# ayotoasset/AdditiveCausalExpansion

Hardware: AMD Instinct MI355X
Metric: log-marg-lik+grad evals/sec at n=16384,d=20; Cholesky GF/s vs MFMA peak (higher is better)
Workload: dtype f64; 1 GPU; C2: n=16384, d=20, Matern32, ns basis B=10, fp64; one para_update (kernel assembly + SPD inverse/log-det + all P gradients + RMSE/evidence + Nadam step) per step; n=16384, p=20, B=10, kernel=Matern32, parallelism=single

## Files before the change

additivecausalexpansion_amd/csrc/ace_sweep.hip:

```cpp
#include "ace_internal.h"

#include "ace_wgtime.h"

namespace ace {

#define CHAIN_PRIO() __builtin_amdgcn_s_setprio(1)


struct PivotLds {
  __attribute__((aligned(16))) double colb[2][SUB];
  __attribute__((aligned(16))) double rowb[2][SUB];
  double pv[SUB];
};

template <int T>
__device__ __forceinline__ double row_bcast(double x) {
  long v = __builtin_bit_cast(long, x);
  long b = __builtin_amdgcn_update_dpp((long)0, v, 0x150 + T, 0xf, 0xf, true);
  return __builtin_bit_cast(double, b);
}

template <int G>
__device__ __forceinline__ double rep_row_bp(double x, int lane) {
  const int addr = ((lane & 15) | (G << 4)) << 2;
// ... 407 lines not shown
      __hip_atomic_fetch_add(ctr + 1, 1, __ATOMIC_RELAXED, __HIP_MEMORY_SCOPE_AGENT) == nwg - 1) {
    __hip_atomic_store(ctr, 0, __ATOMIC_RELAXED, __HIP_MEMORY_SCOPE_AGENT);
    __hip_atomic_store(ctr + 1, 0, __ATOMIC_RELAXED, __HIP_MEMORY_SCOPE_AGENT);
  }
}

#ifndef ACE_BK
#define ACE_BK 16
#endif
constexpr int BK = ACE_BK;
constexpr int LDL = 144;
constexpr int NCH = NB / BK;
constexpr int UTHREADS = 512;
constexpr int SM128 = 2, SH128 = 64;
constexpr int SM64 = 2, SH64 = 32;
static_assert(BK == 16, "staging maps 512 threads x 4 doubles onto a 128 x 16 chunk");

__device__ __forceinline__ void st_a(double *p, double v) { __builtin_nontemporal_store(v, p); }
__device__ __forceinline__ double ld_a(const double *p) { return __builtin_nontemporal_load(p); }

struct GatherOut {
  double *P, *W, *S0;
  int64_t k0, ldp;
  double *low = nullptr, *send = nullptr;
  int64_t h = 0;
  int G = 1;
  int64_t lr0 = 0;
};
static inline GatherOut no_gather() { return GatherOut{nullptr, nullptr, nullptr, -1, 0}; }
static inline GatherOut pack_out(double *low, double *send, double *P, double *W, double *S0,
                                 int64_t k0, int64_t naug, int G) {
  GatherOut g{P, W, S0, k0, naug};
  if (G > 1) {
    g.low = low;
    g.send = send;
  }
  g.h = naug - k0;
  g.G = G;
  return g;
}

__device__ __forceinline__ void gput(const GatherOut &g, int64_t r, int64_t c, double v) {
  if (r < c) return;
  const int64_t cc = c - g.k0, rr = r - g.k0;
  if (g.low) {
    if ((uint64_t)cc < (uint64_t)NB) {
      g.low[(rr - g.lr0) + cc * g.h] = v;
      if ((uint64_t)rr < (uint64_t)NB && r != c) g.low[cc + rr * g.h] = v;
    } else if ((uint64_t)rr < (uint64_t)NB) {
      g.send[(lcol(c, g.G) / NB) * NB * NB + rr + (c % NB) * NB] = v;
    }
  }
  if (!g.P) return;
  if ((uint64_t)cc < (uint64_t)NB) {
    g.P[r + cc * g.ldp] = -v;
    if ((uint64_t)rr < (uint64_t)NB) {
      g.W[r + cc * g.ldp] = v;
      if (rr < SUB) g.S0[rr + cc * SUB] = v;
    }
  }
  if ((uint64_t)rr < (uint64_t)NB && r != c) {
    g.P[c + rr * g.ldp] = -v;
    if ((uint64_t)cc < (uint64_t)NB) {
      g.W[c + rr * g.ldp] = v;
      if (cc < SUB) g.S0[cc + rr * SUB] = v;
    }
  }
}

__device__ __forceinline__ void gput_aug_dead(const GatherOut &g, const double *A, int64_t ld,
                                              int64_t R0, int64_t C0, int tid, int nthr,
                                              int64_t L0 = -1) {
  const int64_t cc0 = C0 - g.k0;
  if ((uint64_t)cc0 >= (uint64_t)NB) return;
  const int64_t lc0 = L0 >= 0 ? L0 : C0;
  for (int e = tid; e < (UT - 16) * UT; e += nthr) {
    const int a = 16 + e % (UT - 16), c = e / (UT - 16);
    const double v = A[(R0 + a) + (lc0 + c) * ld];
    if (g.low) g.low[(R0 + a - g.k0 - g.lr0) + (cc0 + c) * g.h] = v;
    if (g.P) g.P[(R0 + a) + (cc0 + c) * g.ldp] = -v;
  }
}

__global__ __launch_bounds__(UTHREADS, 2) void k_update(double *__restrict__ A, int64_t ld,
                                                        const double *__restrict__ Rop,
                                                        const double *__restrict__ Cop,
                                                        const double *__restrict__ Wk,
                                                        int64_t ldp, int64_t k0, int kx,
                                                        const Tile *__restrict__ tiles, int G,
                                                        GatherOut go) {
  ACE_WGT(6, gridDim.x < 4096 || blockIdx.x % 32 == 0);
  __shared__ __attribute__((aligned(16))) double sW[2][BK][LDL];
  __shared__ __attribute__((aligned(16))) double sP[2][BK][LDL];
  constexpr int KT = NB / UT;
  int I, J;
  if (tiles) {
    const Tile tt = tiles[blockIdx.x];
    I = tt.I;
    J = tt.J;
    if (I < 0) return;
  } else {
    const int t = blockIdx.x;
    int i = (int)((sqrt(8.0 * (double)t + 1.0) - 1.0) * 0.5);
    while ((i + 1) * (i + 2) / 2 <= t) ++i;
    while (i * (i + 1) / 2 > t) --i;
    I = i;
    J = t - i * (i + 1) / 2;
  }
  if (kx >= 0 && ((I >= kx * KT && I < (kx + 1) * KT) || (J >= kx * KT && J < (kx + 1) * KT)))
    return;
  const int kt0 = (int)(k0 / UT), kt1 = kt0 + KT;
  const bool Ik = I >= kt0 && I < kt1, Jk = J >= kt0 && J < kt1;
  const int64_t R0 = (int64_t)I * UT, C0 = (int64_t)J * UT;
  const int64_t L0 = lcol(C0, G);
  const int tid = threadIdx.x;

  if (Ik || Jk) {
    if (Ik && !Jk) {
      double *tileT = &sW[0][0][0];
      for (int sa = 0; sa < 2; ++sa)
        for (int sb = 0; sb < 2; ++sb) {
          __syncthreads();
          for (int e = tid; e < 4096; e += UTHREADS) {
            const int c = e & 63, a = e >> 6;
            tileT[a * 65 + c] = Wk[(C0 + 64 * sb + c) + (R0 - k0 + 64 * sa + a) * ldp];
          }
          __syncthreads();
          for (int e = tid; e < 4096; e += UTHREADS) {
            const int a = e & 63, c = e >> 6;
            const double v = tileT[a * 65 + c];
            A[(R0 + 64 * sa + a) + (L0 + 64 * sb + c) * ld] = v;
            if (go.k0 >= 0) gput(go, R0 + 64 * sa + a, C0 + 64 * sb + c, v);
          }
        }
    } else {
      for (int e = tid; e < UT * UT; e += UTHREADS) {
        const int a = e & (UT - 1), c = e >> 7;
        const double v = Wk[(R0 + a) + (C0 - k0 + c) * ldp];
        A[(R0 + a) + (L0 + c) * ld] = v;
        if (go.k0 >= 0) gput(go, R0 + a, C0 + c, v);
      }
    }
    return;
  }

  const int lane = tid & 63, wv = tid >> 6;
  const int lr = lane & 15, lk = lane >> 4;
  if (R0 >= ld - AUG) {
    d4 acc;
    const int64_t r = R0 + lr;
    const int64_t c = L0 + 16 * wv + lk;
#pragma unroll
    for (int j = 0; j < 4; ++j) acc[j] = ld_a(&A[r + (c + 4 * j) * ld]);
    const double *gr = Rop + R0 + lr + (int64_t)lk * ldp;
    const double *gc = Cop + C0 + 16 * wv + lr + (int64_t)lk * ldp;
    double an = gc[0], bn = gr[0];
    for (int kk = 0; kk < NB / 4; ++kk) {
      const double a = an, bb = bn;
      if (kk + 1 < NB / 4) {
        an = gc[(int64_t)(4 * (kk + 1)) * ldp];
        bn = gr[(int64_t)(4 * (kk + 1)) * ldp];
      }
      acc = __builtin_amdgcn_mfma_f64_16x16x4f64(a, bb, acc, 0, 0, 0);
    }
#pragma unroll
    for (int j = 0; j < 4; ++j) st_a(&A[r + (c + 4 * j) * ld], acc[j]);
    if (go.k0 >= 0) {
#pragma unroll
      for (int j = 0; j < 4; ++j) gput(go, r, C0 + 16 * wv + lk + 4 * j, acc[j]);
      gput_aug_dead(go, A, ld, R0, C0, tid, UTHREADS, L0);
    }
    return;
  }
  const int sk = tid >> 5, sm = (tid & 31) * SM128;
  const int roff = (int)((R0 + sm) + (int64_t)sk * ldp), coff = (int)((C0 + sm) + (int64_t)sk * ldp);
  double2 rw[2], rp[2];
#pragma unroll
  for (int e = 0; e < 2; ++e) {
    rw[e] = *reinterpret_cast<const double2 *>(Rop + roff + SH128 * e);
    rp[e] = *reinterpret_cast<const double2 *>(Cop + coff + SH128 * e);
  }
  __builtin_amdgcn_sched_barrier(0);
  const int wr = wv & 1, wc = wv >> 1;
  d4 acc[2][4];
#pragma unroll
  for (int ci = 0; ci < 2; ++ci)
#pragma unroll
    for (int ri = 0; ri < 4; ++ri) {
      const int64_t r = R0 + 64 * wr + 16 * ri + lr;
      const int64_t c = L0 + 32 * wc + 16 * ci + lk;
#pragma unroll
      for (int j = 0; j < 4; ++j) acc[ci][ri][j] = ld_a(&A[r + (c + 4 * j) * ld]);
    }
#pragma unroll
  for (int e = 0; e < 2; ++e) {
    *reinterpret_cast<double2 *>(&sW[0][sk][sm + SH128 * e]) = rw[e];
    *reinterpret_cast<double2 *>(&sP[0][sk][sm + SH128 * e]) = rp[e];
  }
  __syncthreads();
  for (int ch = 0; ch < NCH; ++ch) {
    const int cur = ch & 1;
    if (ch + 1 < NCH) {
      const int64_t off = (int64_t)(ch + 1) * BK * ldp;
      const double *nw = Rop + off, *np = Cop + off;
#pragma unroll
      for (int e = 0; e < 2; ++e) {
        rw[e] = *reinterpret_cast<const double2 *>(nw + roff + SH128 * e);
        rp[e] = *reinterpret_cast<const double2 *>(np + coff + SH128 * e);
      }
    }
#pragma unroll
    for (int kk = 0; kk < BK / 4; ++kk) {
      double a[2], b[4];
#pragma unroll
      for (int ci = 0; ci < 2; ++ci) a[ci] = sP[cur][4 * kk + lk][32 * wc + 16 * ci + lr];
#pragma unroll
      for (int ri = 0; ri < 4; ++ri) b[ri] = sW[cur][4 * kk + lk][64 * wr + 16 * ri + lr];
#pragma unroll
      for (int ci = 0; ci < 2; ++ci)
#pragma unroll
        for (int ri = 0; ri < 4; ++ri)
          acc[ci][ri] = __builtin_amdgcn_mfma_f64_16x16x4f64(a[ci], b[ri], acc[ci][ri], 0, 0, 0);
    }
    if (ch + 1 < NCH) {
#pragma unroll
      for (int e = 0; e < 2; ++e) {
        *reinterpret_cast<double2 *>(&sW[cur ^ 1][sk][sm + SH128 * e]) = rw[e];
        *reinterpret_cast<double2 *>(&sP[cur ^ 1][sk][sm + SH128 * e]) = rp[e];
      }
    }
    __syncthreads();
  }
#pragma unroll
  for (int ci = 0; ci < 2; ++ci)
#pragma unroll
    for (int ri = 0; ri < 4; ++ri) {
      const int64_t r = R0 + 64 * wr + 16 * ri + lr;
      const int64_t c = L0 + 32 * wc + 16 * ci + lk;
#pragma unroll
      for (int j = 0; j < 4; ++j) st_a(&A[r + (c + 4 * j) * ld], acc[ci][ri][j]);
    }
  if (go.k0 >= 0) {
#pragma unroll
    for (int ci = 0; ci < 2; ++ci)
#pragma unroll
      for (int ri = 0; ri < 4; ++ri)
#pragma unroll
        for (int j = 0; j < 4; ++j)
          gput(go, R0 + 64 * wr + 16 * ri + lr, C0 + 32 * wc + 16 * ci + lk + 4 * j, acc[ci][ri][j]);
  }
}

__global__ __launch_bounds__(UTHREADS, 2) void k_panel_gemm_t(double *__restrict__ W,
                                                              const double *__restrict__ Pn,
                                                              int64_t ldp, int64_t k0, int G,
                                                              int r, int rt0 = 0,
                                                              int rs0 = 1 << 30, int rs1 = 1 << 30) {
  ACE_WGT(3, true);
  __shared__ __attribute__((aligned(16))) double sW[2][BK][LDL];
  __shared__ __attribute__((aligned(16))) double sP[2][BK][LDL];
  int rt = rt0 + (int)blockIdx.x;
  if (rt >= rs0) rt += rs1 - rs0;
  const int64_t R0 = (int64_t)rt * UT, C0 = (int64_t)blockIdx.y * UT;
  if (R0 >= k0 && R0 < k0 + NB) return;
  if (G > 1 && !owns_col(R0, G, r) && !(owns_col(k0, G, r) && R0 >= k0)) return;
  const int tid = threadIdx.x, lane = tid & 63, wv = tid >> 6;
  const int lr = lane & 15, lk = lane >> 4;
  const int sk = tid >> 5, sm = (tid & 31) * SM128;
  const double *gW = Pn + (R0 + sm) + (int64_t)sk * ldp;
  const double *gP = W + (k0 + C0 + sm) + (int64_t)sk * ldp;
  const int wr = wv & 1, wc = wv >> 1;
  d4 acc[2][4];
#pragma unroll
  for (int ci = 0; ci < 2; ++ci)
#pragma unroll
    for (int ri = 0; ri < 4; ++ri) acc[ci][ri] = d4{0.0, 0.0, 0.0, 0.0};
  double2 w00, w01, p00, p01;
#define PG_LOAD(W0, W1, P0, P1, CH)                                               \
  do {                                                                            \
    const int64_t off_ = (int64_t)(CH) * BK * ldp;                                \
    W0 = *reinterpret_cast<const double2 *>(gW + off_);                           \
    W1 = *reinterpret_cast<const double2 *>(gW + off_ + SH128);                   \
    P0 = *reinterpret_cast<const double2 *>(gP + off_);                           \
    P1 = *reinterpret_cast<const double2 *>(gP + off_ + SH128);                   \
  } while (0)
#define PG_STAGE(W0, W1, P0, P1, BUF)                                             \
  do {                                                                            \
    *reinterpret_cast<double2 *>(&sW[BUF][sk][sm]) = W0;                          \
    *reinterpret_cast<double2 *>(&sW[BUF][sk][sm + SH128]) = W1;                  \
    *reinterpret_cast<double2 *>(&sP[BUF][sk][sm]) = P0;                          \
    *reinterpret_cast<double2 *>(&sP[BUF][sk][sm + SH128]) = P1;                  \
  } while (0)
  auto mma = [&](int cur) {
#pragma unroll
    for (int kk = 0; kk < BK / 4; ++kk) {
      double a[2], b[4];
#pragma unroll
      for (int ci = 0; ci < 2; ++ci) a[ci] = sP[cur][4 * kk + lk][32 * wc + 16 * ci + lr];
#pragma unroll
      for (int ri = 0; ri < 4; ++ri) b[ri] = sW[cur][4 * kk + lk][64 * wr + 16 * ri + lr];
#pragma unroll
      for (int ci = 0; ci < 2; ++ci)
#pragma unroll
        for (int ri = 0; ri < 4; ++ri)
          acc[ci][ri] = __builtin_amdgcn_mfma_f64_16x16x4f64(a[ci], b[ri], acc[ci][ri], 0, 0, 0);
    }
  };
  {
    PG_LOAD(w00, w01, p00, p01, 0);
    PG_STAGE(w00, w01, p00, p01, 0);
    __syncthreads();
    ACE_WGT_MARK(0);
    for (int ch = 0; ch < NCH; ++ch) {
      const int cur = ch & 1;
      if (ch + 1 < NCH) PG_LOAD(w00, w01, p00, p01, ch + 1);
      mma(cur);
      if (ch + 1 < NCH) PG_STAGE(w00, w01, p00, p01, cur ^ 1);
      __syncthreads();
    }
  }
#undef PG_LOAD
#undef PG_STAGE
  ACE_WGT_MARK(1);
#pragma unroll
  for (int ci = 0; ci < 2; ++ci)
#pragma unroll
    for (int ri = 0; ri < 4; ++ri) {
      const int64_t rr = R0 + 64 * wr + 16 * ri + lr;
      const int64_t c = C0 + 32 * wc + 16 * ci + lk;
#pragma unroll
      for (int j = 0; j < 4; ++j) W[rr + (c + 4 * j) * ldp] = acc[ci][ri][j];
    }
}

struct PanelSet {
  const double *R[4];
  const double *C[4];
};
__device__ __forceinline__ const double *psel(const double *const (&p)[4], int j) {
  return j == 0 ? p[0] : j == 1 ? p[1] : j == 2 ? p[2] : p[3];
}

template <bool SH, bool OPQ = false>
__device__ __forceinline__ void update_multi_tile(int I, int J, double (&sW)[2][BK][LDL],
                                                  double (&sP)[2][BK][LDL], double *__restrict__ A,
                                                  int64_t ld, const PanelSet &ps, int npan,
                                                  int64_t ldp, int64_t ka0, const GatherOut &go,
                                                  int G) {
  constexpr int KT = NB / UT;
  const int ta0 = (int)(ka0 / UT);
  const int di = I - ta0, dj = J - ta0;
  const int bi = (di >= 0 && di < npan * KT) ? di / KT : -1;
  const int bj = (dj >= 0 && dj < npan * KT) ? dj / KT : -1;
  const int jm = bi > bj ? bi : bj;
  const int64_t R0 = (int64_t)I * UT, C0 = (int64_t)J * UT;
  const int64_t L0 = SH ? lcol(C0, G) : C0;
  int tid = threadIdx.x;
  if (OPQ) __asm__ volatile("" : "+v"(tid));
  const double *const(&WS)[4] = SH ? ps.C : ps.R;

  if (jm == npan - 1) {
    const double *Wl = psel(WS, jm);
    const int64_t kl0 = ka0 + (int64_t)jm * NB;
    if (bi == jm && bj != jm) {
      double *tileT = &sW[0][0][0];
      for (int sa = 0; sa < 2; ++sa)
        for (int sb = 0; sb < 2; ++sb) {
          __syncthreads();
          for (int e = tid; e < 4096; e += UTHREADS) {
            const int c = e & 63, a = e >> 6;
            tileT[a * 65 + c] = Wl[(C0 + 64 * sb + c) + (R0 - kl0 + 64 * sa + a) * ldp];
          }
          __syncthreads();
          for (int e = tid; e < 4096; e += UTHREADS) {
            const int a = e & 63, c = e >> 6;
            const double v = tileT[a * 65 + c];
            A[(R0 + 64 * sa + a) + (L0 + 64 * sb + c) * ld] = v;
            if (go.k0 >= 0) gput(go, R0 + 64 * sa + a, C0 + 64 * sb + c, v);
          }
        }
    } else {
      for (int e = tid; e < UT * UT; e += UTHREADS) {
        const int a = e & (UT - 1), c = e >> 7;
        const double v = Wl[(R0 + a) + (C0 - kl0 + c) * ldp];
        A[(R0 + a) + (L0 + c) * ld] = v;
        if (go.k0 >= 0) gput(go, R0 + a, C0 + c, v);
      }
    }
    return;
  }
  const bool from_w = jm >= 0;
  const int seg0 = from_w ? jm + 1 : 0;
  const bool jin = bj == jm;
  const int64_t wrs = jin ? 1 : ldp, wcs = jin ? ldp : 1;
  const double *wab = from_w ? psel(WS, jm) - (ka0 + (int64_t)jm * NB) * ldp : nullptr;

  const int lane = tid & 63, wv = tid >> 6;
  const int lr = lane & 15, lk = lane >> 4;
  if (R0 >= ld - AUG) {
    d4 acc;
    const int64_t r = R0 + lr;
    const int64_t c = C0 + 16 * wv + lk, lc = L0 + 16 * wv + lk;
#pragma unroll
    for (int j = 0; j < 4; ++j)
      acc[j] = from_w ? wab[r * wrs + (c + 4 * j) * wcs] : ld_a(&A[r + (lc + 4 * j) * ld]);
    for (int pnl = seg0; pnl < npan; ++pnl) {
      const double *gr = psel(ps.R, pnl) + R0 + lr + (int64_t)lk * ldp;
      const double *gc = psel(ps.C, pnl) + C0 + 16 * wv + lr + (int64_t)lk * ldp;
      double an = gc[0], bn = gr[0];
      for (int kk = 0; kk < NB / 4; ++kk) {
        const double a = an, bb = bn;
        if (kk + 1 < NB / 4) {
          an = gc[(int64_t)(4 * (kk + 1)) * ldp];
          bn = gr[(int64_t)(4 * (kk + 1)) * ldp];
        }
        acc = __builtin_amdgcn_mfma_f64_16x16x4f64(a, bb, acc, 0, 0, 0);
      }
    }
#pragma unroll
    for (int j = 0; j < 4; ++j) st_a(&A[r + (lc + 4 * j) * ld], acc[j]);
    if (go.k0 >= 0) {
#pragma unroll
      for (int j = 0; j < 4; ++j) gput(go, r, c + 4 * j, acc[j]);
      gput_aug_dead(go, A, ld, R0, C0, tid, UTHREADS, L0);
    }
    return;
  }
  constexpr int SMU = SH ? 4 : SM128, SHU = SH ? 2 : SH128;
  const int sk = tid >> 5, sm = (tid & 31) * SMU;
  const int roff = (int)((R0 + sm) + (int64_t)sk * ldp), coff = (int)((C0 + sm) + (int64_t)sk * ldp);
  double2 rw0, rw1, rp0, rp1;
  {
    const double *w = psel(ps.R, seg0) + roff, *pp = psel(ps.C, seg0) + coff;
    rw0 = *reinterpret_cast<const double2 *>(w);
    rw1 = *reinterpret_cast<const double2 *>(w + SHU);
    rp0 = *reinterpret_cast<const double2 *>(pp);
    rp1 = *reinterpret_cast<const double2 *>(pp + SHU);
  }
  __builtin_amdgcn_sched_barrier(0);
  const int wr = wv & 1, wc = wv >> 1;
  d4 acc[2][4];
#pragma unroll
  for (int ci = 0; ci < 2; ++ci)
#pragma unroll
    for (int ri = 0; ri < 4; ++ri) {
      const int64_t r = R0 + 64 * wr + 16 * ri + lr;
      const int64_t c = C0 + 32 * wc + 16 * ci + lk, lc = L0 + 32 * wc + 16 * ci + lk;
      if (from_w) {
#pragma unroll
        for (int j = 0; j < 4; ++j) acc[ci][ri][j] = wab[r * wrs + (c + 4 * j) * wcs];
      } else {
#pragma unroll
        for (int j = 0; j < 4; ++j) acc[ci][ri][j] = ld_a(&A[r + (lc + 4 * j) * ld]);
      }
    }
  *reinterpret_cast<double2 *>(&sW[0][sk][sm]) = rw0;
  *reinterpret_cast<double2 *>(&sW[0][sk][sm + SHU]) = rw1;
  *reinterpret_cast<double2 *>(&sP[0][sk][sm]) = rp0;
  *reinterpret_cast<double2 *>(&sP[0][sk][sm + SHU]) = rp1;
  __syncthreads();
  for (int seg = seg0; seg < npan; ++seg) {
    const double *sw = psel(ps.R, seg), *sp = psel(ps.C, seg);
    const bool last = seg + 1 == npan;
    const double *nxw = last ? sw : psel(ps.R, seg + 1);
    const double *nxp = last ? sp : psel(ps.C, seg + 1);
    for (int ch = 0; ch < NCH; ++ch) {
      const int cur = ch & 1;
      const bool more = ch + 1 < NCH || !last;
      if (more) {
        const double *nw = (ch + 1 < NCH ? sw + (int64_t)(ch + 1) * BK * ldp : nxw) + roff;
        const double *np = (ch + 1 < NCH ? sp + (int64_t)(ch + 1) * BK * ldp : nxp) + coff;
        rw0 = *reinterpret_cast<const double2 *>(nw);
        rw1 = *reinterpret_cast<const double2 *>(nw + SHU);
        rp0 = *reinterpret_cast<const double2 *>(np);
        rp1 = *reinterpret_cast<const double2 *>(np + SHU);
      }
#pragma unroll
      for (int kk = 0; kk < BK / 4; ++kk) {
        double a[2], b[4];
#pragma unroll
        for (int ci = 0; ci < 2; ++ci) a[ci] = sP[cur][4 * kk + lk][32 * wc + 16 * ci + lr];
#pragma unroll
        for (int ri = 0; ri < 4; ++ri) b[ri] = sW[cur][4 * kk + lk][64 * wr + 16 * ri + lr];
#pragma unroll
        for (int ci = 0; ci < 2; ++ci)
#pragma unroll
          for (int ri = 0; ri < 4; ++ri)
            acc[ci][ri] = __builtin_amdgcn_mfma_f64_16x16x4f64(a[ci], b[ri], acc[ci][ri], 0, 0, 0);
      }
      if (more) {
        *reinterpret_cast<double2 *>(&sW[cur ^ 1][sk][sm]) = rw0;
        *reinterpret_cast<double2 *>(&sW[cur ^ 1][sk][sm + SHU]) = rw1;
        *reinterpret_cast<double2 *>(&sP[cur ^ 1][sk][sm]) = rp0;
        *reinterpret_cast<double2 *>(&sP[cur ^ 1][sk][sm + SHU]) = rp1;
      }
      __syncthreads();
    }
  }
#pragma unroll
  for (int ci = 0; ci < 2; ++ci)
#pragma unroll
    for (int ri = 0; ri < 4; ++ri) {
      const int64_t r = R0 + 64 * wr + 16 * ri + lr;
      const int64_t lc = L0 + 32 * wc + 16 * ci + lk;
#pragma unroll
      for (int j = 0; j < 4; ++j) st_a(&A[r + (lc + 4 * j) * ld], acc[ci][ri][j]);
    }
  if (go.k0 >= 0) {
#pragma unroll
    for (int ci = 0; ci < 2; ++ci)
#pragma unroll
      for (int ri = 0; ri < 4; ++ri)
#pragma unroll
// ... 237 lines not shown
  const int lr = lane & 15, lk = lane >> 4;
#pragma unroll
  for (int ci = 0; ci < QT / 32; ++ci)
#pragma unroll
    for (int ri = 0; ri < QT / 32; ++ri) {
      const int64_t r = R0 + QT / 2 * wr + 16 * ri + lr;
      const int64_t c = C0 + QT / 2 * wc + 16 * ci + lk;
#pragma unroll
      for (int j = 0; j < 4; ++j) fn(r, c + 4 * j, acc[ci][ri][j]);
    }
}

template <int QT, class Load, class Primed>
__device__ __forceinline__ void q_pipeline(d4 (&acc)[QT / 32][QT / 32], double (*sW)[BK][QT + 8],
                                           double (*sP)[BK][QT + 8], int T, Load load,
                                           Primed primed) {
  static_assert(NCH % 2 == 0 && NCH >= 4, "two chunks per pipeline turn");
  const int tid = threadIdx.x;
  const int lane = tid & 63, wv = tid >> 6;
  const int wr = wv & 1, wc = wv >> 1;
  const int lr = lane & 15, lk = lane >> 4;
  const int sk = tid >> 4, sm = (tid & 15) * SM64;
  auto stage = [&](QChunk<QT> c, int buf) {
#pragma unroll
    for (int e = 0; e < QT / 32; ++e)
      *reinterpret_cast<double2 *>(&sW[buf][sk][sm + QT / 2 * e]) = c.w[e];
#pragma unroll
    for (int e = 0; e < QT / 32; ++e)
      *reinterpret_cast<double2 *>(&sP[buf][sk][sm + QT / 2 * e]) = c.p[e];
  };
  auto mma = [&](int cur) {
#pragma unroll
    for (int kk = 0; kk < BK / 4; ++kk) {
      double a[QT / 32], b[QT / 32];
#pragma unroll
      for (int ci = 0; ci < QT / 32; ++ci) a[ci] = sP[cur][4 * kk + lk][QT / 2 * wc + 16 * ci + lr];
#pragma unroll
      for (int ri = 0; ri < QT / 32; ++ri) b[ri] = sW[cur][4 * kk + lk][QT / 2 * wr + 16 * ri + lr];
#pragma unroll
      for (int ci = 0; ci < QT / 32; ++ci)
#pragma unroll
        for (int ri = 0; ri < QT / 32; ++ri)
          acc[ci][ri] = __builtin_amdgcn_mfma_f64_16x16x4f64(a[ci], b[ri], acc[ci][ri], 0, 0, 0);
    }
  };
  QChunk<QT> c0 = load(0);
  stage(c0, 0);
  QChunk<QT> c1 = load(1);
  c0 = load(2);
  __syncthreads();
  primed();
#pragma unroll 1
  for (int t = 0; t < T; t += 2) {
    mma(0);
    stage(c1, 1);
    if (t + 3 < T) c1 = load(t + 3);
    __syncthreads();
    mma(1);
    if (t + 2 < T) {
      stage(c0, 0);
      if (t + 4 < T) c0 = load(t + 4);
    }
    __syncthreads();
  }
}

template <int QT>
__device__ __forceinline__ void update_q(double *__restrict__ A, int64_t ld, const PanelSet &ps,
                                         int npan, int64_t ldp, const Tile *__restrict__ tiles,
                                         const GatherOut &go, double *__restrict__ pivSW,
                                         double *__restrict__ piv, int *__restrict__ flag,
                                         int *__restrict__ qctr) {
  ACE_WGT(4, true);
  constexpr int QL = QT + 8;
  constexpr int NPC = (XT / QT) * (XT / QT);
  constexpr int NS = 2 * 2 * BK * QL > SUB * (SUB + 2) ? 2 * 2 * BK * QL : SUB * (SUB + 2);
  __shared__ __attribute__((aligned(16))) double sbuf[NS];
  double (*sW)[BK][QL] = reinterpret_cast<double (*)[BK][QL]>(sbuf);
  double (*sP)[BK][QL] = reinterpret_cast<double (*)[BK][QL]>(sbuf + 2 * BK * QL);
  const Tile tt = tiles[blockIdx.x / (4 * NPC)];
  if (tt.I < 0) return;
  const int q = (blockIdx.x / NPC) & 3, pc = blockIdx.x % NPC;
  const int64_t Rq = (int64_t)tt.I * UT + XT * (q & 1), Cq = (int64_t)tt.J * UT + XT * (q >> 1);
  const int64_t R0 = Rq + QT * (pc & 1), C0 = Cq + QT * (pc >> 1);
  const int tid = threadIdx.x;
  const int lane = tid & 63, wv = tid >> 6;
  const int wr = wv & 1, wc = wv >> 1;
  const int lr = lane & 15, lk = lane >> 4;
  d4 acc[QT / 32][QT / 32];
#pragma unroll
  for (int ci = 0; ci < QT / 32; ++ci)
#pragma unroll
    for (int ri = 0; ri < QT / 32; ++ri) {
      const int64_t r = R0 + QT / 2 * wr + 16 * ri + lr;
      const int64_t c = C0 + QT / 2 * wc + 16 * ci + lk;
#pragma unroll
      for (int j = 0; j < 4; ++j) acc[ci][ri][j] = A[r + (c + 4 * j) * ld];
    }
  const int sk = tid >> 4, sm = (tid & 15) * SM64;
  q_pipeline<QT>(
      acc, sW, sP, npan * NCH,
      [=](int t) {
        const int pj = t / NCH, ch = t - pj * NCH;
        const int64_t off = (int64_t)ch * BK * ldp;
        return q_load<QT>(psel(ps.R, pj) + (R0 + sm) + (int64_t)sk * ldp + off,
                          psel(ps.C, pj) + (C0 + sm) + (int64_t)sk * ldp + off);
      },
      [] {});
  ACE_WGT_MARK(0);
#pragma unroll
  for (int ci = 0; ci < QT / 32; ++ci)
#pragma unroll
    for (int ri = 0; ri < QT / 32; ++ri) {
      const int64_t r = R0 + QT / 2 * wr + 16 * ri + lr;
      const int64_t c = C0 + QT / 2 * wc + 16 * ci + lk;
#pragma unroll
      for (int j = 0; j < 4; ++j) {
        const double v = acc[ci][ri][j];
        A[r + (c + 4 * j) * ld] = v;
        if (go.k0 >= 0) gput(go, r, c + 4 * j, v);
      }
    }
  if (!(pivSW && go.k0 >= 0 && Rq == go.k0 && Cq == go.k0)) return;
  __shared__ double pv[SUB];
  double(*M)[SUB + 2] = reinterpret_cast<double(*)[SUB + 2]>(sbuf);
  double v[SUB / 4];
  if constexpr (QT == XT) {
    q_each<QT>(acc, 0, 0, [&](int64_t a, int64_t c, double x) {
      if (a >= c) {
        M[a][c] = x;
        M[c][a] = x;
      }
    });
    __syncthreads();
#pragma unroll
    for (int qq = 0; qq < SUB / 4; ++qq) v[qq] = M[lane][16 * wv + qq];
  } else {
    __shared__ int last;
    asm volatile("s_waitcnt vmcnt(0)" ::: "memory");
    __syncthreads();
    if (tid == 0) {
      __builtin_amdgcn_fence(__ATOMIC_RELEASE, "agent");
      last = __hip_atomic_fetch_add(qctr, 1, __ATOMIC_RELAXED, __HIP_MEMORY_SCOPE_AGENT) == NPC - 1;
      if (last) {
        __builtin_amdgcn_fence(__ATOMIC_ACQUIRE, "agent");
        __hip_atomic_store(qctr, 0, __ATOMIC_RELAXED, __HIP_MEMORY_SCOPE_AGENT);
      }
    }
    __syncthreads();
    if (!last) return;
#pragma unroll
    for (int qq = 0; qq < SUB / 4; ++qq)
      v[qq] = __hip_atomic_load(go.S0 + lane + (16 * wv + qq) * SUB, __ATOMIC_RELAXED,
                                __HIP_MEMORY_SCOPE_AGENT);
  }
  ACE_WGT_MARK(1);
  pivot_sweep_blk<SUB + 2>(v, M, pv, tid);
  ACE_WGT_MARK(2);
  pivot_store(v, pv, tid, pivSW, piv, go.k0, flag);
}
__global__ __launch_bounds__(256, 4) void k_update_q(double *__restrict__ A, int64_t ld, PanelSet ps,
                                                  int npan, int64_t ldp,
                                                  const Tile *__restrict__ tiles, GatherOut go,
                                                  double *__restrict__ pivSW,
                                                  double *__restrict__ piv,
                                                  int *__restrict__ flag) {
// ... 561 lines not shown
```

additivecausalexpansion_amd/csrc/ace_sweep_plan.cpp:

```cpp
#include "ace_sweep_plan.h"

#include <map>

namespace ace {

double tile_list_work(const std::vector<Tile> &tl, int64_t nT, int64_t ta0, int npan, int kx0,
                      int kx1) {
  double cnt = 0.0;
  for (const Tile &t : tl)
    if (t.I >= 0) cnt += tile_work(t, nT, ta0, npan, kx0, kx1);
  return cnt;
}

double update_gemm_tiles(int64_t naug, int64_t k0, int kx, bool look) {
  const int nT = (int)(naug / UT);
  double cnt = 0.0;
  for (int I = 0; I < nT; ++I)
    for (int J = 0; J <= I; ++J)
      if (const Tile t{I, J}; in_blocks(t, kx, kx + 1) == look) cnt += tile_work(t, nT, k0 / UT, 1, -1, -1);
  return cnt;
}

double update_gemm_tiles_group(int64_t naug, int64_t ka0, int npan, int kx0, int kx1) {
  const int nT = (int)(naug / UT);
  double cnt = 0.0;
  for (int I = 0; I < nT; ++I)
    for (int J = 0; J <= I; ++J) cnt += tile_work(Tile{I, J}, nT, ka0 / UT, npan, kx0, kx1);
  return cnt;
}

double sweep_flops(int64_t naug, int64_t npad) {
  thread_local int64_t cn = -1, cp = -1;
  thread_local double cf = 0.0;
  if (naug == cn && npad == cp) return cf;
  double f = 0.0;
  for (int64_t k0 = 0; k0 < npad; k0 += NB)
    f += update_gemm_tiles(naug, k0, -1, false) * TILE_FLOPS +
         2.0 * (double)(naug - NB) * NB * NB;
  cn = naug;
  cp = npad;
  cf = f;
  return f;
}

std::vector<Tile> cross_update_tiles(int64_t naug, int steps, int S, std::vector<int64_t> &off) {
  const std::vector<Tile> lower = own_tiles(naug / UT, UT, 1, 0);
  std::vector<Tile> all;
  off.assign(1, 0);
  for (int k = 0; k + 1 < steps; ++k) {
    std::vector<Tile> t;
    for (const Tile &x : lower)
      if (in_blocks(x, k + 1, k + 2)) t.push_back(x);
    const std::vector<Tile> o = S > 0 ? xcd_update_order(t, S) : t;
    all.insert(all.end(), o.begin(), o.end());
    off.push_back((int64_t)all.size());
  }
  return all;
}

std::vector<Tile> pair_bulk_orders(int64_t naug, int steps, int S, int64_t *len, int G, int r,
                                   int Z) {
  const int64_t nT = naug / UT;
  constexpr int KT = NB / UT;
  const int ng = (steps + Z - 1) / Z;
  const std::vector<Tile> base = own_tiles(nT, UT, G, r);
  std::vector<Tile> all;
  std::vector<std::vector<Tile>> lists;
  *len = 0;
  for (int g = 0; g < ng; ++g) {
    const int z = std::min(Z, steps - Z * g);
    const int64_t ta0 = (int64_t)Z * g * KT;
    const bool more = g + 1 < ng;
    const int kx0 = more ? Z * (g + 1) : -1, kx1 = more ? std::min(Z * (g + 1) + Z, steps) : -1;
    auto cost = [&](const Tile &t) -> double {
      const double w = tile_work(t, nT, ta0, z, kx0, kx1);
      return w > 0.0 ? w : in_blocks(t, kx0, kx1) ? 0.0 : 0.05;
    };
    lists.push_back(xcd_update_order(base, std::max(1, S), cost));
    *len = std::max<int64_t>(*len, (int64_t)lists.back().size());
  }
  for (auto &o : lists) {
    o.resize((size_t)*len, Tile{-1, -1});
    all.insert(all.end(), o.begin(), o.end());
  }
  return all;
}

std::vector<Tile> group_head_tiles(int64_t naug, int steps, int Z, int S,
                                   std::vector<int64_t> &off) {
  const std::vector<Tile> lower = own_tiles(naug / UT, UT, 1, 0);
  constexpr int KT = NB / UT;
  const int ng = (steps + Z - 1) / Z;
  std::vector<Tile> all;
  off.assign((size_t)ng * 2 * Z + 1, 0);
  for (int G = 0; G < ng; ++G) {
    const int kb = Z * G, z = std::min(Z, steps - kb);
    std::vector<std::vector<Tile>> L((size_t)2 * Z);
    for (const Tile &t : lower) {
      const int bi = t.I / KT - kb, bj = t.J / KT - kb;
      const bool ii = bi >= 0 && bi < z, ij = bj >= 0 && bj < z;
      if (ii && ij) {
        L[0].push_back(t);
        for (int i = 0; i + 1 < z; ++i)
          if (bj >= i + 1) L[(size_t)(2 + i)].push_back(t);
      } else if (ii || ij) {
        L[1].push_back(t);
      }
      for (int j = 1; j < z; ++j) {
        if (bi != j && bj != j) continue;
        const bool head = bj == j && bi >= j && bi < z;
        if (!head) L[(size_t)(z + j)].push_back(t);
      }
    }
    for (int m = 0; m < 2 * Z; ++m) {
      const std::vector<Tile> o = S > 0 ? xcd_update_order(L[(size_t)m], S) : L[(size_t)m];
      all.insert(all.end(), o.begin(), o.end());
      off[(size_t)G * 2 * Z + m + 1] = (int64_t)all.size();
    }
  }
  return all;
}

std::vector<Tile> rank_head_tiles(int64_t naug, int steps, int Z, int S, int G, int r,
                                  std::vector<int64_t> &off) {
  std::vector<int64_t> all_off;
  const std::vector<Tile> all = group_head_tiles(naug, steps, Z, S, all_off);
  std::vector<Tile> mine;
  off.assign(all_off.size(), 0);
  for (size_t m = 0; m + 1 < all_off.size(); ++m) {
    for (int64_t i = all_off[m]; i < all_off[m + 1]; ++i)
      if (const Tile &t = all[(size_t)i]; t.I >= 0 && owns_col((int64_t)t.J * UT, G, r)) mine.push_back(t);
    off[m + 1] = (int64_t)mine.size();
  }
  return mine;
}

std::vector<Tile> rank_asm_tiles(int64_t npad, int Z, int G, int r, int64_t *nfirst) {
  std::vector<Tile> t = own_tiles(npad / AT, AT, G, r);
  *nfirst = std::stable_partition(t.begin(), t.end(), [&](const Tile &x) { return x.J < Z * NB / AT; }) - t.begin();
  return t;
}

std::vector<Tile> rank_grad_tiles(int64_t n, int G, int r, int64_t *ndiag) {
  std::vector<Tile> t = own_tiles((n + AT - 1) / AT, AT, G, r);
  *ndiag = std::stable_partition(t.begin(), t.end(), [](const Tile &x) { return x.I == x.J; }) - t.begin();
  return t;
}

std::vector<Tile> grad_tile_order(int64_t n, int S, const uint32_t *mask, int64_t *ndiag) {
  const int64_t ntr = (n + AT - 1) / AT;
  std::vector<Tile> lst, low;
  for (int64_t I = 0; I < ntr; ++I)
    for (int64_t J = 0; J <= I; ++J) (J == I ? lst : low).push_back(Tile{(int)I, (int)J});
  std::function<double(const Tile &)> cost;
  if (mask)
    cost = [mask](const Tile &t) { return 1.0 + __builtin_popcount(mask[t.I] & mask[t.J]); };
  const std::vector<Tile> o = xcd_update_order(low, S, cost);
  lst.insert(lst.end(), o.begin(), o.end());
  *ndiag = ntr;
  return lst;
}

double tile_list_pairs(const std::vector<Tile> &tl) {
  double pairs = 0.0;
  for (const Tile &t : tl)
    if (t.I >= 0) pairs += t.I == t.J ? AT * (AT + 1) / 2 : AT * AT;
  return pairs;
}

std::vector<Tile> own_tiles(int64_t ntile, int T, int G, int r) {
  std::vector<Tile> t;
  for (int64_t I = 0; I < ntile; ++I)
    for (int64_t J = 0; J <= I; ++J)
      if (owns_col(J * T, G, r)) t.push_back(Tile{(int)I, (int)J});
  return t;
}

std::vector<Tile> xcd_update_order(const std::vector<Tile> &tl, int S,
                                   const std::function<double(const Tile &)> &cost) {
  constexpr int X = 8;
  std::vector<std::vector<Tile>> q(X);
  std::map<std::pair<int, int>, std::vector<Tile>> sb;
  for (const Tile &t : tl) sb[{t.I / S, t.J / S}].push_back(t);
  for (auto &kv : sb) {
    int x = 0;
    for (int i = 1; i < X; ++i)
      if (q[i].size() < q[x].size()) x = i;
    q[x].insert(q[x].end(), kv.second.begin(), kv.second.end());
  }
  if (cost)
    for (auto &v : q)
      std::stable_sort(v.begin(), v.end(),
                       [&](const Tile &a, const Tile &b) { return cost(a) > cost(b); });
  size_t len = 0;
  for (auto &v : q) len = std::max(len, v.size());
  std::vector<Tile> out(len * X, Tile{-1, -1});
  for (int x = 0; x < X; ++x)
    for (size_t i = 0; i < q[x].size(); ++i) out[i * X + x] = q[x][i];
  return out;
}

}
```

additivecausalexpansion_amd/csrc/ace_sweep_plan.h:

```cpp
#pragma once
#include <stdint.h>

#include <algorithm>
#include <functional>
#include <vector>

namespace ace {

#ifndef ACE_NB
#define ACE_NB 256
#endif
constexpr int NB = ACE_NB;
constexpr int SUB = 64;
constexpr int UT = 128;
constexpr int AUG = 128;
constexpr int AT = 64;
constexpr double TILE_FLOPS = 2.0 * UT * UT * NB;

#ifdef __HIPCC__
__host__ __device__
#endif
inline __attribute__((always_inline)) bool owns_col(int64_t c, int G, int r) {
  return G == 1 || (c / NB) % G == r;
}
inline int64_t ncols_local(int64_t naug, int G, int r) { return ((naug + NB - 1) / NB - r + G - 1) / G * NB; }
inline int shard_row_slots(int k, int G) { return (k + G - 1) / G; }

struct Tile {
  int I, J;
};

inline bool in_blocks(const Tile &t, int k0, int k1) {
  constexpr int KT = NB / UT;
  return k0 >= 0 && ((t.I >= k0 * KT && t.I < k1 * KT) || (t.J >= k0 * KT && t.J < k1 * KT));
}
inline int tile_first_panel(const Tile &t, int64_t ta0, int npan, int kx0, int kx1) {
  constexpr int KT = NB / UT;
  if (in_blocks(t, kx0, kx1)) return npan;
  const int64_t di = t.I - ta0, dj = t.J - ta0;
  const int bi = (di >= 0 && di < npan * KT) ? (int)(di / KT) : -1;
  const int bj = (dj >= 0 && dj < npan * KT) ? (int)(dj / KT) : -1;
  return std::max(bi, bj) + 1;
}
inline double tile_rows(const Tile &t, int64_t nT) { return t.I == nT - 1 ? 16.0 / UT : 1.0; }
inline double tile_work(const Tile &t, int64_t nT, int64_t ta0, int npan, int kx0, int kx1) {
  return tile_rows(t, nT) * (npan - tile_first_panel(t, ta0, npan, kx0, kx1));
}
double tile_list_work(const std::vector<Tile> &tl, int64_t nT, int64_t ta0, int npan, int kx0,
                      int kx1);
double update_gemm_tiles(int64_t naug, int64_t k0, int kx, bool look);
double update_gemm_tiles_group(int64_t naug, int64_t ka0, int npan, int kx0, int kx1);
double sweep_flops(int64_t naug, int64_t npad);

std::vector<Tile> own_tiles(int64_t ntile, int T, int G, int r);
std::vector<Tile> xcd_update_order(const std::vector<Tile> &tl, int S,
                                   const std::function<double(const Tile &)> &cost = nullptr);
std::vector<Tile> cross_update_tiles(int64_t naug, int steps, int S, std::vector<int64_t> &off);
std::vector<Tile> pair_bulk_orders(int64_t naug, int steps, int S, int64_t *len, int G, int r,
                                   int Z);
std::vector<Tile> group_head_tiles(int64_t naug, int steps, int Z, int S,
                                   std::vector<int64_t> &off);
std::vector<Tile> rank_head_tiles(int64_t naug, int steps, int Z, int S, int G, int r,
                                  std::vector<int64_t> &off);
std::vector<Tile> rank_asm_tiles(int64_t npad, int Z, int G, int r, int64_t *nfirst);
std::vector<Tile> rank_grad_tiles(int64_t n, int G, int r, int64_t *ndiag);
std::vector<Tile> grad_tile_order(int64_t n, int S, const uint32_t *mask, int64_t *ndiag);

double tile_list_pairs(const std::vector<Tile> &tl);
inline double asm_flops(double pairs, double B, double p) { return pairs * B * (3 * p + 3); }
inline double grad_flops(double pairs, double B, double p, bool matern) {
  return pairs * (4 * B * p + 2 * p) + (matern ? pairs * B * p : 0);
}

struct SweepEvents {
  int steps, Z;
  int groups() const { return (steps + Z - 1) / Z; }
  int ready() const { return 0; }
  int tail_after() const { return 1; }
  int filler() const { return 2; }
  int bulk_done(int g) const { return 4 + g; }
  int head_done(int g) const { return group0() + 4 * g; }
  int tail_done(int g) const { return group0() + 4 * g + 1; }
  int q_done(int g) const { return group0() + 4 * g + 2; }
  int last_tail(int g) const { return group0() + 4 * g + 3; }
  int substeps_done(int k) const { return panel0() + 2 * k; }
  int head_gemm_done(int k) const { return panel0() + 2 * k + 1; }
  int step_panel_done(int k) const { return step0() + 2 * k; }
  int step_bulk_before(int k) const { return step0() + 2 * k + 1; }
  int bulk_before(int g) const { return before0() + g; }
  int count() const { return before0() + groups(); }

 private:
  int group0() const { return 4 + groups(); }
  int panel0() const { return group0() + 4 * groups(); }
  int step0() const { return panel0() + 2 * steps; }
  int before0() const { return step0() + 2 * steps; }
};

#ifndef ACE_BULK_RESERVE_N
#define ACE_BULK_RESERVE_N 8192
#endif
inline bool small_n(int64_t naug) { return naug <= ACE_BULK_RESERVE_N + AUG; }
inline int default_group(int64_t naug) { return small_n(naug) ? 3 : 4; }
inline int default_bulk_reserve(int64_t naug) { return small_n(naug) ? 1 : 0; }
inline bool default_q_first(int64_t naug) { return small_n(naug); }
constexpr int BQ_INTS = 2 + 64;
struct BqLayout {
  int64_t fctr, qctr, ints;
};
inline BqLayout bq_layout(int steps, int Z) {
  const int64_t q = (int64_t)((steps + Z - 1) / Z) * BQ_INTS;
  return BqLayout{q, q + 2 * steps, q + 3 * steps};
}

}
```

Measured before the change: 14.23 evals/s.

## Compute only lower-triangular blocks on diagonal trailing-update tiles

Adds a dedicated diagonal-tile path for the Cholesky trailing update. Each of 8 waves computes a balanced share of the 36 lower-triangular 16x16 subblocks (4 or 5 per wave), instead of the full 128x128 tile. The quadrant update kernel also skips strictly upper quadrants. The aim is to cut wasted MFMA work on the symmetric diagonal, at the cost of an extra code path, register pressure and possible wave imbalance.

```diff
diff --git a/additivecausalexpansion_amd/csrc/ace_sweep.hip b/additivecausalexpansion_amd/csrc/ace_sweep.hip
--- a/additivecausalexpansion_amd/csrc/ace_sweep.hip
+++ b/additivecausalexpansion_amd/csrc/ace_sweep.hip
@@ -513,6 +513,136 @@
   }
 }
 
+struct DiagDeal {
+  int s, h;
+  __device__ __forceinline__ explicit DiagDeal(int tid) {
+    const int wv = __builtin_amdgcn_readfirstlane(tid >> 6);
+    s = wv & 3;
+    h = wv >> 2;
+  }
+  __device__ __forceinline__ bool has(int q) const { return q < 4 || !h; }
+  __device__ __forceinline__ bool low(int q) const { return h && q <= s; }
+  __device__ __forceinline__ int brow(int q) const { return low(q) ? s : 7 - s; }
+  __device__ __forceinline__ int bcol(int q) const { return !h || q <= s ? q : q + 4 - s; }
+};
+__device__ __forceinline__ void diag_mma(d4 (&acc)[5], const DiagDeal &d, const double (&sW)[BK][LDL],
+                                         const double (&sP)[BK][LDL], int lr, int lk) {
+#pragma unroll
+  for (int kk = 0; kk < BK / 4; ++kk) {
+    double a[4];
+#pragma unroll
+    for (int q = 0; q < 4; ++q) a[q] = sP[4 * kk + lk][16 * d.bcol(q) + lr];
+    const double bl = sW[4 * kk + lk][16 * d.brow(0) + lr], bh = sW[4 * kk + lk][16 * (7 - d.s) + lr];
+#pragma unroll
+    for (int q = 0; q < 4; ++q)
+      acc[q] = __builtin_amdgcn_mfma_f64_16x16x4f64(a[q], d.low(q) ? bl : bh, acc[q], 0, 0, 0);
+  }
+  if (d.has(4)) {
+    double a[BK / 4], b[BK / 4];
+#pragma unroll
+    for (int kk = 0; kk < BK / 4; ++kk) {
+      a[kk] = sP[4 * kk + lk][16 * 4 + lr];
+      b[kk] = sW[4 * kk + lk][16 * (7 - d.s) + lr];
+    }
+#pragma unroll
+    for (int kk = 0; kk < BK / 4; ++kk)
+      acc[4] = __builtin_amdgcn_mfma_f64_16x16x4f64(a[kk], b[kk], acc[4], 0, 0, 0);
+  }
+}
+
+struct PanelSet {
+  const double *R[4];
+  const double *C[4];
+};
+__device__ __forceinline__ const double *psel(const double *const (&p)[4], int j) {
+  return j == 0 ? p[0] : j == 1 ? p[1] : j == 2 ? p[2] : p[3];
+}
+
+template <int SMU, int SHU>
+__device__ __forceinline__ void update_diag_tile(int tid, double (&sW)[2][BK][LDL], double (&sP)[2][BK][LDL],
+                                                 double *__restrict__ A, int64_t ld, int64_t R0,
+                                                 int64_t C0, int64_t L0, const PanelSet &ps, int seg0,
+                                                 int npan, int64_t ldp, const double *wab,
+                                                 int64_t wrs, int64_t wcs, const GatherOut &go) {
+  const bool from_w = wab != nullptr;
+  __asm__ volatile("" : "+v"(tid));
+  const int lane = tid & 63, lr = lane & 15, lk = lane >> 4;
+  const int sk = tid >> 5, sm = (tid & 31) * SMU;
+  const int roff = (int)((R0 + sm) + (int64_t)sk * ldp), coff = (int)((C0 + sm) + (int64_t)sk * ldp);
+  double2 rw0, rw1, rp0, rp1;
+  {
+    const double *w = psel(ps.R, seg0) + roff, *pp = psel(ps.C, seg0) + coff;
+    rw0 = *reinterpret_cast<const double2 *>(w);
+    rw1 = *reinterpret_cast<const double2 *>(w + SHU);
+    rp0 = *reinterpret_cast<const double2 *>(pp);
+    rp1 = *reinterpret_cast<const double2 *>(pp + SHU);
+  }
+  __builtin_amdgcn_sched_barrier(0);
+  const DiagDeal dd(tid);
+  const unsigned la = lr + lk * (unsigned)ld, la4 = 4 * (unsigned)ld;
+  d4 dacc[5];
+#pragma unroll
+  for (int q = 0; q < 5; ++q)
+    if (dd.has(q)) {
+      const int64_t rq = R0 + 16 * dd.brow(q), cq = 16 * dd.bcol(q);
+      if (from_w) {
+        const double *src = wab + rq * wrs + (C0 + cq) * wcs;
+        const unsigned lw = lr * (unsigned)wrs + lk * (unsigned)wcs, lw4 = 4 * (unsigned)wcs;
+#pragma unroll
+        for (int j = 0; j < 4; ++j) dacc[q][j] = src[lw + j * lw4];
+      } else {
+        const double *src = A + rq + (L0 + cq) * ld;
+#pragma unroll
+        for (int j = 0; j < 4; ++j) dacc[q][j] = ld_a(&src[la + j * la4]);
+      }
+    }
+  *reinterpret_cast<double2 *>(&sW[0][sk][sm]) = rw0;
+  *reinterpret_cast<double2 *>(&sW[0][sk][sm + SHU]) = rw1;
+  *reinterpret_cast<double2 *>(&sP[0][sk][sm]) = rp0;
+  *reinterpret_cast<double2 *>(&sP[0][sk][sm + SHU]) = rp1;
+  __syncthreads();
+  for (int seg = seg0; seg < npan; ++seg) {
+    const double *sw = psel(ps.R, seg), *sp = psel(ps.C, seg);
+    const bool last = seg + 1 == npan;
+    const double *nxw = last ? sw : psel(ps.R, seg + 1);
+    const double *nxp = last ? sp : psel(ps.C, seg + 1);
+#pragma unroll 1
+    for (int ch = 0; ch < NCH; ++ch) {
+      const int cur = ch & 1;
+      const bool more = ch + 1 < NCH || !last;
+      if (more) {
+        const double *nw = (ch + 1 < NCH ? sw + (int64_t)(ch + 1) * BK * ldp : nxw) + roff;
+        const double *np = (ch + 1 < NCH ? sp + (int64_t)(ch + 1) * BK * ldp : nxp) + coff;
+        rw0 = *reinterpret_cast<const double2 *>(nw);
+        rw1 = *reinterpret_cast<const double2 *>(nw + SHU);
+        rp0 = *reinterpret_cast<const double2 *>(np);
+        rp1 = *reinterpret_cast<const double2 *>(np + SHU);
+      }
+      diag_mma(dacc, dd, sW[cur], sP[cur], lr, lk);
+      if (more) {
+        *reinterpret_cast<double2 *>(&sW[cur ^ 1][sk][sm]) = rw0;
+        *reinterpret_cast<double2 *>(&sW[cur ^ 1][sk][sm + SHU]) = rw1;
+        *reinterpret_cast<double2 *>(&sP[cur ^ 1][sk][sm]) = rp0;
+        *reinterpret_cast<double2 *>(&sP[cur ^ 1][sk][sm + SHU]) = rp1;
+      }
+      __syncthreads();
+    }
+  }
+  const bool gk = go.k0 >= 0 && (uint64_t)(C0 - go.k0) < (uint64_t)NB;
+#pragma unroll
+  for (int q = 0; q < 5; ++q)
+    if (dd.has(q)) {
+      const int64_t rq = R0 + 16 * dd.brow(q), cq = 16 * dd.bcol(q);
+      double *dst = A + rq + (L0 + cq) * ld;
+#pragma unroll
+      for (int j = 0; j < 4; ++j) st_a(&dst[la + j * la4], dacc[q][j]);
+      if (gk) {
+#pragma unroll
+        for (int j = 0; j < 4; ++j) gput(go, rq + lr, C0 + cq + lk + 4 * j, dacc[q][j]);
+      }
+    }
+}
+
 __global__ __launch_bounds__(UTHREADS, 2) void k_update(double *__restrict__ A, int64_t ld,
                                                         const double *__restrict__ Rop,
                                                         const double *__restrict__ Cop,
@@ -603,6 +733,13 @@
     }
     return;
   }
+  if (I == J) {
+    const PanelSet ps{{Rop, Rop, Rop, Rop}, {Cop, Cop, Cop, Cop}};
+    const double *nw = nullptr;
+    __asm__ volatile("" : "+s"(nw));
+    update_diag_tile<SM128, SH128>(tid, sW, sP, A, ld, R0, C0, L0, ps, 0, 1, ldp, nw, 1, ldp, go);
+    return;
+  }
   const int sk = tid >> 5, sm = (tid & 31) * SM128;
   const int roff = (int)((R0 + sm) + (int64_t)sk * ldp), coff = (int)((C0 + sm) + (int64_t)sk * ldp);
   double2 rw[2], rp[2];
@@ -762,14 +899,6 @@
 #pragma unroll
       for (int j = 0; j < 4; ++j) W[rr + (c + 4 * j) * ldp] = acc[ci][ri][j];
     }
-}
-
-struct PanelSet {
-  const double *R[4];
-  const double *C[4];
-};
-__device__ __forceinline__ const double *psel(const double *const (&p)[4], int j) {
-  return j == 0 ? p[0] : j == 1 ? p[1] : j == 2 ? p[2] : p[3];
 }
 
 template <bool SH, bool OPQ = false>
@@ -860,6 +989,10 @@
   constexpr int SMU = SH ? 4 : SM128, SHU = SH ? 2 : SH128;
   const int sk = tid >> 5, sm = (tid & 31) * SMU;
   const int roff = (int)((R0 + sm) + (int64_t)sk * ldp), coff = (int)((C0 + sm) + (int64_t)sk * ldp);
+  if (OPQ ? __builtin_amdgcn_readfirstlane(I == J) != 0 : I == J) {
+    update_diag_tile<SMU, SHU>(tid, sW, sP, A, ld, R0, C0, L0, ps, seg0, npan, ldp, wab, wrs, wcs, go);
+    return;
+  }
   double2 rw0, rw1, rp0, rp1;
   {
     const double *w = psel(ps.R, seg0) + roff, *pp = psel(ps.C, seg0) + coff;
@@ -1263,6 +1396,7 @@
   if (tt.I < 0) return;
   const int q = (blockIdx.x / NPC) & 3, pc = blockIdx.x % NPC;
   const int64_t Rq = (int64_t)tt.I * UT + XT * (q & 1), Cq = (int64_t)tt.J * UT + XT * (q >> 1);
+  if (Rq < Cq) return;
   const int64_t R0 = Rq + QT * (pc & 1), C0 = Cq + QT * (pc >> 1);
   const int tid = threadIdx.x;
   const int lane = tid & 63, wv = tid >> 6;
```

Result: no change. 14.28 evals/s (median of 6 runs) (+0.4%).

## Balance XCD tile queues by modeled tile time with swap refinement

Applied to the files above, without the earlier changes.

Tile lists for the Cholesky bulk and head updates are now dealt across the 8 XCD queues by a modeled per-tile time (fixed cost plus per-panel cost, small cost for skipped tiles) instead of by tile count. A local-search refinement then moves or swaps tiles between the heaviest and lighter queues until loads are within a small slack. This targets load imbalance across XCDs at large n, where some queues end up with more panel work than others. It applies only when n is above the small-n threshold, adds host-side planning cost, and relies on hand-set timing constants.

```diff
diff --git a/additivecausalexpansion_amd/csrc/ace_sweep_plan.cpp b/additivecausalexpansion_amd/csrc/ace_sweep_plan.cpp
--- a/additivecausalexpansion_amd/csrc/ace_sweep_plan.cpp
+++ b/additivecausalexpansion_amd/csrc/ace_sweep_plan.cpp
@@ -1,5 +1,6 @@
 #include "ace_sweep_plan.h"
 
+#include <cmath>
 #include <map>
 
 namespace ace {
@@ -76,7 +77,9 @@
       const double w = tile_work(t, nT, ta0, z, kx0, kx1);
       return w > 0.0 ? w : in_blocks(t, kx0, kx1) ? 0.0 : 0.05;
     };
-    lists.push_back(xcd_update_order(base, std::max(1, S), cost));
+    std::function<double(const Tile &)> time;
+    if (!small_n(naug)) time = [&](const Tile &t) { return tile_time(t, nT, ta0, z, kx0, kx1); };
+    lists.push_back(xcd_update_order(base, std::max(1, S), cost, time));
     *len = std::max<int64_t>(*len, (int64_t)lists.back().size());
   }
   for (auto &o : lists) {
@@ -112,8 +115,16 @@
         if (!head) L[(size_t)(z + j)].push_back(t);
       }
     }
+    const int64_t nT = naug / UT;
+    const int zp = std::min(Z, steps - Z * (G - 1));
     for (int m = 0; m < 2 * Z; ++m) {
-      const std::vector<Tile> o = S > 0 ? xcd_update_order(L[(size_t)m], S) : L[(size_t)m];
+      std::function<double(const Tile &)> time;
+      if (!small_n(naug) && m == 1 && G > 0)
+        time = [=](const Tile &t) { return tile_time(t, nT, (int64_t)Z * (G - 1) * KT, zp, -1, -1); };
+      else if (!small_n(naug) && m > z && m < 2 * z)
+        time = [=](const Tile &t) { return tile_time(t, nT, (int64_t)kb * KT, m - z, -1, -1); };
+      const std::vector<Tile> o =
+          S > 0 ? xcd_update_order(L[(size_t)m], S, nullptr, time) : L[(size_t)m];
       all.insert(all.end(), o.begin(), o.end());
       off[(size_t)G * 2 * Z + m + 1] = (int64_t)all.size();
     }
@@ -176,22 +187,81 @@
   return t;
 }
 
+static void refine_deal(std::vector<std::vector<Tile>> &q, std::vector<double> &load,
+                        const std::function<double(const Tile &)> &time) {
+  constexpr double DEAL_SLACK = 1.001;
+  const int X = (int)q.size();
+  std::vector<std::vector<double>> tm((size_t)X);
+  for (int x = 0; x < X; ++x)
+    for (const Tile &t : q[(size_t)x]) tm[(size_t)x].push_back(time(t));
+  for (int it = 0; it < 256; ++it) {
+    int h = 0;
+    double sum = 0.0;
+    for (int i = 0; i < X; ++i) {
+      sum += load[(size_t)i];
+      if (load[(size_t)i] > load[(size_t)h]) h = i;
+    }
+    if (load[(size_t)h] <= DEAL_SLACK * sum / X) break;
+    std::vector<int> by_load((size_t)X);
+    for (int i = 0; i < X; ++i) by_load[(size_t)i] = i;
+    std::stable_sort(by_load.begin(), by_load.end(),
+                     [&](int a, int b) { return load[(size_t)a] < load[(size_t)b]; });
+    int l = -1, ba = -1, bb = -1;
+    for (int c = 0; c < X && ba < 0; ++c) {
+      l = by_load[(size_t)c];
+      const double gap = load[(size_t)h] - load[(size_t)l];
+      double best = gap / 2 * (1.0 - 1e-9);
+      for (int a = 0; a < (int)tm[(size_t)h].size(); ++a) {
+        const double ta = tm[(size_t)h][(size_t)a];
+        if (const double e = std::abs(ta - gap / 2); e < best) best = e, ba = a, bb = -1;
+        for (int b = 0; b < (int)tm[(size_t)l].size(); ++b)
+          if (const double e = std::abs(ta - tm[(size_t)l][(size_t)b] - gap / 2); e < best)
+            best = e, ba = a, bb = b;
+      }
+    }
+    if (ba < 0) break;
+    std::vector<Tile> &qh = q[(size_t)h], &ql = q[(size_t)l];
+    std::vector<double> &th = tm[(size_t)h], &tl = tm[(size_t)l];
+    double d = th[(size_t)ba];
+    if (bb >= 0) {
+      d -= tl[(size_t)bb];
+      std::swap(qh[(size_t)ba], ql[(size_t)bb]);
+      std::swap(th[(size_t)ba], tl[(size_t)bb]);
+    } else {
+      ql.push_back(qh[(size_t)ba]);
+      tl.push_back(th[(size_t)ba]);
+      qh.erase(qh.begin() + ba);
+      th.erase(th.begin() + ba);
+    }
+    load[(size_t)h] -= d;
+    load[(size_t)l] += d;
+  }
+}
+
 std::vector<Tile> xcd_update_order(const std::vector<Tile> &tl, int S,
-                                   const std::function<double(const Tile &)> &cost) {
+                                   const std::function<double(const Tile &)> &cost,
+                                   const std::function<double(const Tile &)> &time) {
   constexpr int X = 8;
   std::vector<std::vector<Tile>> q(X);
+  std::vector<double> load(X, 0.0);
   std::map<std::pair<int, int>, std::vector<Tile>> sb;
   for (const Tile &t : tl) sb[{t.I / S, t.J / S}].push_back(t);
   for (auto &kv : sb) {
     int x = 0;
     for (int i = 1; i < X; ++i)
-      if (q[i].size() < q[x].size()) x = i;
+      if (load[i] < load[x] || (load[i] == load[x] && q[i].size() < q[x].size())) x = i;
     q[x].insert(q[x].end(), kv.second.begin(), kv.second.end());
-  }
+    if (time)
+      for (const Tile &t : kv.second) load[x] += time(t);
+  }
+  if (time) refine_deal(q, load, time);
   if (cost)
-    for (auto &v : q)
-      std::stable_sort(v.begin(), v.end(),
-                       [&](const Tile &a, const Tile &b) { return cost(a) > cost(b); });
+    for (auto &v : q) {
+      std::vector<std::pair<double, Tile>> kv;
+      for (const Tile &t : v) kv.push_back({cost(t), t});
+      std::stable_sort(kv.begin(), kv.end(), [](const auto &a, const auto &b) { return a.first > b.first; });
+      for (size_t i = 0; i < v.size(); ++i) v[i] = kv[i].second;
+    }
   size_t len = 0;
   for (auto &v : q) len = std::max(len, v.size());
   std::vector<Tile> out(len * X, Tile{-1, -1});
diff --git a/additivecausalexpansion_amd/csrc/ace_sweep_plan.h b/additivecausalexpansion_amd/csrc/ace_sweep_plan.h
--- a/additivecausalexpansion_amd/csrc/ace_sweep_plan.h
+++ b/additivecausalexpansion_amd/csrc/ace_sweep_plan.h
@@ -46,6 +46,11 @@
 inline double tile_work(const Tile &t, int64_t nT, int64_t ta0, int npan, int kx0, int kx1) {
   return tile_rows(t, nT) * (npan - tile_first_panel(t, ta0, npan, kx0, kx1));
 }
+constexpr double TILE_SKIP_US = 2.0, TILE_FIXED_US = 48.0, TILE_PANEL_US = 45.0;
+inline double tile_time(const Tile &t, int64_t nT, int64_t ta0, int npan, int kx0, int kx1) {
+  return in_blocks(t, kx0, kx1) ? TILE_SKIP_US
+                                : TILE_FIXED_US + TILE_PANEL_US * tile_work(t, nT, ta0, npan, kx0, kx1);
+}
 double tile_list_work(const std::vector<Tile> &tl, int64_t nT, int64_t ta0, int npan, int kx0,
                       int kx1);
 double update_gemm_tiles(int64_t naug, int64_t k0, int kx, bool look);
@@ -54,7 +59,8 @@
 
 std::vector<Tile> own_tiles(int64_t ntile, int T, int G, int r);
 std::vector<Tile> xcd_update_order(const std::vector<Tile> &tl, int S,
-                                   const std::function<double(const Tile &)> &cost = nullptr);
+                                   const std::function<double(const Tile &)> &cost = nullptr,
+                                   const std::function<double(const Tile &)> &time = nullptr);
 std::vector<Tile> cross_update_tiles(int64_t naug, int steps, int S, std::vector<int64_t> &off);
 std::vector<Tile> pair_bulk_orders(int64_t naug, int steps, int S, int64_t *len, int G, int r,
                                    int Z);
```

Result: no change. 14.05 evals/s before, 14.07 evals/s after (median of 2 runs) (+0.2%).
